# redmod-team/SympGPR

Hardware: AMD Instinct MI355X
Metric: Gram-build GB/s + Cholesky fp64 TFLOP/s at N=65536 d=2; |alpha-alpha_ref|/|alpha_ref| (higher is better)
Workload: dtype f64

## Files before the change

### include/sympgpr_probe.h

```cpp
#ifndef SYMPGPR_PROBE_H
#define SYMPGPR_PROBE_H
#include <stddef.h>
#ifdef __cplusplus
extern "C" {
#endif

int sgpr_probe_mfma_f64(int waves_per_simd, int iters, double *tflops);
int sgpr_probe_hbm_write(size_t bytes, int reps, double *gbs);
int sgpr_probe_mfma_clock(int nacc, int waves_per_simd, int iters, double *out3);
int sgpr_probe_gemm(int m, int n, int k, int lower, double *out4);
int sgpr_probe_gemm_debug(int bits);
int sgpr_probe_leaf(double *out8);
int sgpr_probe_lat(double *out8);
int sgpr_probe_xcc(int nblocks, int *host_out);
int sgpr_probe_cumask(const unsigned *mask_words, int nwords, int nblocks, int *host_out);

int sgpr_probe_generated_eval(int family, int which, int m, const double *xa, const double *ya,
                              const double *xb, const double *yb, const double *l, int nl, double *out);

int sgpr_probe_queue_plan(int n, int nworkers, int *starts_out, int max_starts, unsigned *tasks_out, int max_tasks,
                          int *counts);
int sgpr_probe_queue_plan_partial(int n, int nworkers, int nq, int *starts_out, int max_starts, unsigned *tasks_out,
                                  int max_tasks, int *counts);
int sgpr_probe_queue_trace_begin(int max_tasks);
// ... 10 lines not shown
                            double beta, double *C, size_t ldc, double alpha2, double *C2, size_t ldc2, void *stream);
int sgpr_probe_strassen2_plan(int m, int n, int k, int lower, long smin, long kslab, long smin2, long kslab2, long scratch_doubles,
                              long long *out, int max_records, int *count);
int sgpr_probe_gemm_nt4_dev(int m, int n, int k, const double *A, size_t lda, const double *B, size_t ldb, double beta, int count,
                            double *const *C, const size_t *ldc, const double *alpha, void *stream);
int sgpr_probe_strassen_rec_plan(int m, int n, int k, int lower, long scratch_doubles, long cfg_out[5], long long *out,
                                 int max_records, int *count);
int sgpr_probe_strassen_rec_scratch(int n, unsigned long long out[2]);
int sgpr_probe_gemm_strassen_rec_dev(int m, int n, int k, double alpha, const double *A, size_t lda, const double *B, size_t ldb,
                                     double beta, double *C, size_t ldc, int lower, void *stream);
int sgpr_probe_strassen_schedule(int m, int n, int k, int lower, long capacity_doubles, long long info[12], long long *out,
                                 int max_records, int *count);
int sgpr_probe_batch_layout(int path, int mode, int d, int reg, int nbatch, int n_pts, int nhyp, unsigned long long out[24]);
unsigned sgpr_probe_map_calls(void);
int sgpr_probe_map_team(int ntest, int n0);

int sgpr_probe_trsm_piece(int ticket, int cap, int strips, int out[5]);
int sgpr_probe_trsm_counts(int strips, int cap, unsigned long long out[2]);

int sgpr_probe_census(int na, int threads_a, int lds_a, int spin_a, const unsigned *mask_a, int nwords_a,
                      int nb, int threads_b, int lds_b, int spin_b, const unsigned *mask_b, int nwords_b,
                      unsigned long long *host_out);

#ifdef __cplusplus
}
#endif
#endif
```

### sympgpr_amd/_lib.py

```python
import ctypes as C
import os

import numpy as np

FAMILIES = {"A": 0, "B": 1, "C": 2, "D": 3, "USER": 4}
K_KERN, K_DXDX0, K_DYDY0, K_DXDY0 = 0, 1, 2, 3
K_DLX, K_DLY = 4, 8
K_DX, K_DY, K_DX0, K_DY0, K_DXDX0DY0, K_DYDY0DY0, K_DXDY0DY0 = 16, 17, 18, 19, 20, 21, 22
G_QQ, G_PQ, G_QP, G_PP, G_ALL, G_LOWER, G_OCML, G_DLX, G_DLY = 1, 2, 4, 8, 15, 16, 32, 64, 128
FIT_LOWER_ONLY, FIT_REG, FIT_BLOCK_QQ, FIT_BLOCK_PP = 1, 4, 8, 16
MAP_WRAP_Q, MAP_WRAP_P, MAP_EXPLICIT, MAP_LOSS_NEGP = 1, 2, 4, 8
E_ARG, E_NODEVICE, E_HIP, E_NOMEM, E_STATE = -1, -2, -3, -4, -5
LOO_LPD, LOO_PRESS = 0, 1

ABI_VERSION = 5
_dp = C.POINTER(C.c_double)
_vp = C.c_void_p


class SympGPRError(RuntimeError):
    code = None
    detail = ""


# ... 141 lines not shown
    "sgpr_probe_queue_postmortem": (C.c_int, [C.c_int]),
    "sgpr_probe_queue_force_giveup": (C.c_int, [C.c_int]),
    "sgpr_probe_tune": (C.c_int, [C.c_char_p, C.c_double]),
    "sgpr_probe_map_calls": (C.c_uint, []),
    "sgpr_probe_map_team": (C.c_int, [C.c_int, C.c_int]),
    "sgpr_probe_trsm_piece": (C.c_int, [C.c_int, C.c_int, C.c_int, C.POINTER(C.c_int)]),
    "sgpr_probe_trsm_counts": (C.c_int, [C.c_int, C.c_int, C.POINTER(C.c_ulonglong)]),
    "sgpr_probe_queue_trace_clear": (C.c_int, []),
    "sgpr_probe_strassen_plan": (C.c_int, [C.c_int, C.c_int, C.c_int, C.c_int, C.c_long, C.c_long, C.c_long,
                                           C.POINTER(C.c_longlong), C.c_int, C.POINTER(C.c_int)]),
    "sgpr_probe_gemm_strassen_dev": (C.c_int, [C.c_int, C.c_int, C.c_int, C.c_double, C.c_void_p, C.c_size_t, C.c_void_p, C.c_size_t,
                                               C.c_double, C.c_void_p, C.c_size_t, C.c_int, C.c_void_p]),
    "sgpr_probe_gemm_nt2_dev": (C.c_int, [C.c_int, C.c_int, C.c_int, C.c_double, C.c_void_p, C.c_size_t, C.c_void_p, C.c_size_t,
                                          C.c_double, C.c_void_p, C.c_size_t, C.c_double, C.c_void_p, C.c_size_t, C.c_void_p]),
    "sgpr_probe_strassen2_plan": (C.c_int, [C.c_int, C.c_int, C.c_int, C.c_int, C.c_long, C.c_long, C.c_long, C.c_long, C.c_long,
                                            C.POINTER(C.c_longlong), C.c_int, C.POINTER(C.c_int)]),
    "sgpr_probe_strassen_rec_plan": (C.c_int, [C.c_int, C.c_int, C.c_int, C.c_int, C.c_long, C.POINTER(C.c_long),
                                               C.POINTER(C.c_longlong), C.c_int, C.POINTER(C.c_int)]),
    "sgpr_probe_strassen_rec_scratch": (C.c_int, [C.c_int, C.POINTER(C.c_ulonglong)]),
    "sgpr_probe_strassen_schedule": (C.c_int, [C.c_int, C.c_int, C.c_int, C.c_int, C.c_long, C.POINTER(C.c_longlong),
                                               C.POINTER(C.c_longlong), C.c_int, C.POINTER(C.c_int)]),
    "sgpr_probe_gemm_strassen_rec_dev": (C.c_int, [C.c_int, C.c_int, C.c_int, C.c_double, C.c_void_p, C.c_size_t, C.c_void_p, C.c_size_t,
                                                   C.c_double, C.c_void_p, C.c_size_t, C.c_int, C.c_void_p]),
    "sgpr_probe_gemm_nt4_dev": (C.c_int, [C.c_int, C.c_int, C.c_int, C.c_void_p, C.c_size_t, C.c_void_p, C.c_size_t, C.c_double, C.c_int,
                                          C.POINTER(C.c_void_p), C.POINTER(C.c_size_t), C.POINTER(C.c_double), C.c_void_p]),
    "sgpr_probe_batch_layout": (C.c_int, [C.c_int, C.c_int, C.c_int, C.c_int, C.c_int, C.c_int, C.c_int,
                                          C.POINTER(C.c_ulonglong)]),
    "sgpr_probe_census": (C.c_int, [C.c_int, C.c_int, C.c_int, C.c_int, C.POINTER(C.c_uint), C.c_int,
                                    C.c_int, C.c_int, C.c_int, C.c_int, C.POINTER(C.c_uint), C.c_int,
                                    C.POINTER(C.c_ulonglong)]),
}

_LIB = None
_PROBE = None


def load_library():
    global _LIB
    if _LIB is not None:
        return _LIB
    path = lib_path()
    if os.environ.get("SYMPGPR_NO_TORCH_PRELOAD") != "1":
        try:
            import torch
        except ImportError:
            pass
# ... 78 lines not shown
```

### sympgpr_amd/csrc/chol.hip

```cpp
#include <algorithm>
#include <cstdlib>
#include <mutex>
#include <vector>

#include "cholq.h"
#include "common.h"
#include "gemm_tile.h"
#include "leaf.h"

namespace sgpr {

namespace {

using namespace leaf;


__global__ __launch_bounds__(LT) void leaf_kernel(int nb, double *A, size_t lda, double *inv,
                                                  int *dinfo, int goff, int mode,
                                                  unsigned long long *stamps)
{
    __shared__ double s[LEAF_LDS];
    if (nb == LEAF) leaf_body(s, (int)LEAF, A, lda, inv, dinfo, goff, mode, stamps);
    else            leaf_body(s, nb, A, lda, inv, dinfo, goff, mode, stamps);
}
// ... 753 lines not shown
    a.inv = q.inv + (size_t)p * q.stride_inv + (size_t)(q.k0 / (int)LEAF) * LEAF * LEAF;
    a.dinfo = q.info + p; a.goff = q.k0;
    a.flags = q.flags + (size_t)p * PFLAG_STRIDE;
    a.below_early = 1;
    (void)panel_strip(a, g, s, sh);
}

inline int split(int n)
{
    int n1 = ((n / 2 + LEAF - 1) / LEAF) * LEAF;
    if (n1 >= n) n1 -= LEAF;
    return n1;
}

struct Ctx {
    double *inv;
    int *dinfo;
    hipStream_t st;
    int la_max = 0;
    int *flags = nullptr;
    void *qws = nullptr;
    bool strassen = false;
    StrassenRec rec;
};

int potrf_lookahead(int n, double *A, size_t lda, const Ctx &c, int nb, int off0);
inline int la_block(int n) { return n <= 4096 ? 256 : (n <= 24576 ? 512 : (n <= 40960 ? 1024 : 2048)); }

int trsm_rec(int m, int n, const double *L, size_t ldl, double *B, size_t ldb, int off, const Ctx &c)
{
    if (n <= LEAF) {
        return gemm_nt(m, n, n, 1.0, B, ldb, c.inv + (size_t)(off / LEAF) * LEAF * LEAF, LEAF, 0.0,
                       B, ldb, 0, 0, c.st);
    }
    const int n1 = split(n), n2 = n - n1;
    int rc = trsm_rec(m, n1, L, ldl, B, ldb, off, c);
    if (rc) return rc;
    if (c.strassen) rc = gemm_nt_strassen_cfg(m, n2, n1, -1.0, B, ldb, L + n1, ldl, 1.0, B + (size_t)n1 * ldb, ldb, 0, strassen_rec_cfg(c.rec, n1, 0), c.st);
    else            rc = gemm_nt(m, n2, n1, -1.0, B, ldb, L + n1, ldl, 1.0, B + (size_t)n1 * ldb, ldb, 0, 0, c.st);
    if (rc) return rc;
    return trsm_rec(m, n2, L + n1 + (size_t)n1 * ldl, ldl, B + (size_t)n1 * ldb, ldb, off + n1, c);
}

int trsm_rl_rec(int m, int n, const double *L, size_t ldl, double *B, size_t ldb, int off, const Ctx &c)
{
    if (n <= LEAF)
        return gemm_nn(m, n, n, 1.0, B, ldb, c.inv + (size_t)(off / LEAF) * LEAF * LEAF, LEAF, 0.0, B, ldb, c.st);
    const int n1 = split(n), n2 = n - n1;
    int rc = trsm_rl_rec(m, n2, L + n1 + (size_t)n1 * ldl, ldl, B + (size_t)n1 * ldb, ldb, off + n1, c);
    if (rc) return rc;
    rc = gemm_nn(m, n1, n2, -1.0, B + (size_t)n1 * ldb, ldb, L + n1, ldl, 1.0, B, ldb, c.st);
    if (rc) return rc;
    return trsm_rl_rec(m, n1, L, ldl, B, ldb, off, c);
}

int potrf_rec(int n, double *A, size_t lda, int off, const Ctx &c)
{
    if (n <= LEAF) {
        hipLaunchKernelGGL(leaf_kernel, dim3(1), dim3(LT), 0, c.st, n, A, lda,
                           c.inv + (size_t)(off / LEAF) * LEAF * LEAF, c.dinfo, off, (int)LEAF_FACTOR,
                           (unsigned long long *)nullptr);
        SGPR_CHECK_LAUNCH();
        return 0;
    }
    if (n > 4 * LEAF && n <= c.la_max) return potrf_lookahead(n, A, lda, c, 0, off);
    const int n1 = split(n), n2 = n - n1;
    double *A21 = A + n1, *A22 = A + n1 + (size_t)n1 * lda;
    int rc = potrf_rec(n1, A, lda, off, c);
    if (rc) return rc;
    rc = trsm_rec(n2, n1, A, lda, A21, lda, off, c);
    if (rc) return rc;
    if (c.strassen) rc = gemm_nt_strassen_cfg(n2, n2, n1, -1.0, A21, lda, A21, lda, 1.0, A22, lda, 1, strassen_rec_cfg(c.rec, n1, 1), c.st);
    else            rc = gemm_nt(n2, n2, n1, -1.0, A21, lda, A21, lda, 1.0, A22, lda, 1, 0, c.st);
    if (rc) return rc;
    return potrf_rec(n2, A22, lda, off + n1, c);
}

int trsv_n_rec(int n, const double *L, size_t ldl, double *b, int off, const Ctx &c)
{
    if (n <= LEAF) {
        hipLaunchKernelGGL(leaf_matvec_kernel, dim3(1), dim3(MV_T), 0, c.st, n,
                           c.inv + (size_t)(off / LEAF) * LEAF * LEAF, b, 0);
        SGPR_CHECK_LAUNCH();
        return 0;
    }
    if (n <= TRSV_BLOCK) {
        hipLaunchKernelGGL(trsv_block_kernel, dim3(1), dim3(MV_T), 0, c.st, n, L, ldl,
                           c.inv + (size_t)(off / LEAF) * LEAF * LEAF, b, 0);
        SGPR_CHECK_LAUNCH();
        return 0;
    }
    const int n1 = split(n), n2 = n - n1;
    int rc = trsv_n_rec(n1, L, ldl, b, off, c);
    if (rc) return rc;
    rc = gemv_n_sub(n2, n1, L + n1, ldl, b, b + n1, c.st);
// ... 110 lines not shown
    int dev = -1;
    if (caller) {
        SGPR_HIP(hipStreamGetDevice(caller, &dev));
    } else {
        SGPR_HIP(hipGetDevice(&dev));
    }
    if (dev < 0 || dev >= 64) { set_error("potrf: device index out of range"); return SGPR_E_ARG; }
    std::lock_guard<std::mutex> lock(g_side_mu);
    if (!side[dev]) {
        int cur = -1, lo = 0, hi = 0;
        SGPR_HIP(hipGetDevice(&cur));
        if (cur != dev) SGPR_HIP(hipSetDevice(dev));
        hipError_t e = hipDeviceGetStreamPriorityRange(&lo, &hi);
        if (e == hipSuccess) e = hipStreamCreateWithPriority(&side[dev], hipStreamNonBlocking, hi);
        if (e == hipSuccess) register_exit_release();
        if (cur != dev) (void)hipSetDevice(cur);
        SGPR_HIP(e);
    }
    *out = side[dev];
    *dev_out = dev;
    return 0;
}

hipStream_t g_sum[64][2] = {};
}

int strassen_sum_streams(hipStream_t caller, int count, hipStream_t *out)
{
    int dev = -1;
    if (caller) {
        SGPR_HIP(hipStreamGetDevice(caller, &dev));
    } else {
        SGPR_HIP(hipGetDevice(&dev));
    }
    if (dev < 0 || dev >= 64 || count < 1 || count > 2) { set_error("strassen_sum_streams: bad device or count"); return SGPR_E_ARG; }
    std::lock_guard<std::mutex> lock(g_side_mu);
    for (int t = 0; t < count; ++t) {
        if (!g_sum[dev][t]) {
            int cur = -1, lo = 0, hi = 0;
            SGPR_HIP(hipGetDevice(&cur));
            if (cur != dev) SGPR_HIP(hipSetDevice(dev));
            hipError_t e = hipDeviceGetStreamPriorityRange(&lo, &hi);
            if (e == hipSuccess) e = hipStreamCreateWithPriority(&g_sum[dev][t], hipStreamNonBlocking, lo);
            if (e == hipSuccess) register_exit_release();
            if (cur != dev) (void)hipSetDevice(cur);
            SGPR_HIP(e);
        }
        out[t] = g_sum[dev][t];
    }
    return 0;
}

namespace {

struct QueueDevice {
    std::mutex mu;
    hipEvent_t done = nullptr;
    int ncu = 0;
    hipStream_t workers[4] = {}, panels[4] = {};
    bool overlap_ok[4] = {};
    bool failed = false;
};
QueueDevice g_qdev[64];

__global__ void overlap_probe_kernel(int *w, int me)
{
    __hip_atomic_store((gint *)(w + me), 1, __ATOMIC_RELAXED, __HIP_MEMORY_SCOPE_AGENT);
    const unsigned long long t0 = __builtin_amdgcn_s_memrealtime();
    int seen = 0;
    while (!(seen = __hip_atomic_load((gint *)(w + 1 - me), __ATOMIC_RELAXED, __HIP_MEMORY_SCOPE_AGENT))) {
        __builtin_amdgcn_s_sleep(32);
        if (__builtin_amdgcn_s_memrealtime() - t0 > 5000000ull) break;
// ... 122 lines not shown
    cholq::remember(ws, n, (int)(plan->tasks.size() / 2));
    cholq::remember_plan(plan);
    static const bool qdebug = tune("q_debug", 0) != 0;
    if (qdebug) {
        SGPR_HIP(hipStreamSynchronize(su));
        cholq::postmortem(false);
    }
    if (plan->nq < plan->nblk) {
        const int S = plan->starts[plan->nq];
        Ctx ct = c;
        ct.qws = nullptr;
        static const bool nosync = tune("q_nosync", 0) != 0;
        if (!nosync) SGPR_HIP(hipStreamSynchronize(su));
        return potrf_lookahead(n - S, A + S + (size_t)S * lda, lda, ct, 0, off0 + S);
    }
    return 0;
}

void release_all_streams_at_exit()
{
    int ndev = 0;
    if (hipGetDeviceCount(&ndev) != hipSuccess) { (void)hipGetLastError(); return; }
    for (int dev = 0; dev < ndev && dev < 64; ++dev) {
        hipStream_t drop[11] = {};
        int nd = 0;
        {
            std::lock_guard<std::mutex> lock(g_side_mu);
            if (g_side[dev]) { drop[nd++] = g_side[dev]; g_side[dev] = nullptr; }
            for (hipStream_t &s : g_sum[dev]) if (s) { drop[nd++] = s; s = nullptr; }
        }
        {
            QueueDevice &qd = g_qdev[dev];
            std::lock_guard<std::mutex> lock(qd.mu);
            for (int r = 0; r < 4; ++r) {
                if (qd.workers[r]) { drop[nd++] = qd.workers[r]; qd.workers[r] = nullptr; }
                if (qd.panels[r]) { drop[nd++] = qd.panels[r]; qd.panels[r] = nullptr; }
            }
            qd.failed = true;
        }
        if (!nd) continue;
        int cur = -1;
        (void)hipGetDevice(&cur);
        if (cur != dev) (void)hipSetDevice(dev);
        for (int q = 0; q < nd; ++q) (void)hipStreamDestroy(drop[q]);
        if (cur != dev && cur >= 0) (void)hipSetDevice(cur);
    }
    (void)hipGetLastError();
}

int release_streams(int dev)
{
    {
        bool any = false;
        {
            std::lock_guard<std::mutex> lock(g_side_mu);
            any = g_side[dev] != nullptr || g_sum[dev][0] != nullptr || g_sum[dev][1] != nullptr;
        }
        QueueDevice &qd = g_qdev[dev];
        std::lock_guard<std::mutex> lock(qd.mu);
        for (int r = 0; r < 4; ++r) any = any || qd.workers[r] || qd.panels[r];
        any = any || qd.done;
        if (!any) return 0;
    }
    int cur = -1;
    SGPR_HIP(hipGetDevice(&cur));
    if (cur != dev) SGPR_HIP(hipSetDevice(dev));
    hipError_t first = hipSuccess;
    auto drop = [&](hipStream_t &s) {
        if (!s) return;
        hipError_t e = hipStreamSynchronize(s);
        if (e == hipSuccess) e = hipStreamDestroy(s);
        if (e != hipSuccess && first == hipSuccess) first = e;
        s = nullptr;
    };
    {
        std::lock_guard<std::mutex> lock(g_side_mu);
        drop(g_side[dev]);
        drop(g_sum[dev][0]);
        drop(g_sum[dev][1]);
    }
    {
        QueueDevice &qd = g_qdev[dev];
        std::lock_guard<std::mutex> lock(qd.mu);
        for (int r = 0; r < 4; ++r) { drop(qd.workers[r]); drop(qd.panels[r]); }
        if (qd.done) {
            const hipError_t e = hipEventDestroy(qd.done);
            if (e != hipSuccess && first == hipSuccess) first = e;
            qd.done = nullptr;
        }
        qd.ncu = 0;
        qd.failed = false;
        for (int r = 0; r < 4; ++r) qd.overlap_ok[r] = false;
    }
    if (cur != dev) (void)hipSetDevice(cur);
    SGPR_HIP(first);
    return 0;
}

int potrf_lookahead(int n, double *A, size_t lda, const Ctx &c, int nb, int off0)
{
    if (nb == 0 && c.qws && c.flags && cholq::eligible(n) && (lda & 1) == 0 && (((uintptr_t)A & 15) == 0) && off0 % LEAF == 0) {
        const int rq = potrf_queue(n, A, lda, c, off0);
// ... 205 lines not shown
namespace {
int la_max_value()
{
    static const int v = [] { const char *e = getenv("SGPR_LA_MAX"); return (int)tune("la_max", e ? atoi(e) : 57344); }();
    return v;
}
void need_trsm(int m, int n, const StrassenRec &v, int levels, size_t &need)
{
    if (n <= LEAF || std::min(m, n) < 256) return;
    const int n1 = split(n), n2 = n - n1;
    need_trsm(m, n1, v, levels, need);
    need = std::max(need, strassen_scratch_doubles_cfg(m, n2, n1, 0, levels, strassen_rec_cfg(v, n1, 0)));
    need_trsm(m, n2, v, levels, need);
}
void need_potrf(int n, int la_max, const StrassenRec &v, int levels, size_t &need)
{
    if (n <= LEAF || (n > 4 * LEAF && n <= la_max)) return;
    const int n1 = split(n), n2 = n - n1;
    need_potrf(n1, la_max, v, levels, need);
    need_trsm(n2, n1, v, levels, need);
    need = std::max(need, strassen_scratch_doubles_cfg(n2, n2, n1, 1, levels, strassen_rec_cfg(v, n1, 1)));
    need_potrf(n2, la_max, v, levels, need);
}
}

void potrf_strassen_need(int n, size_t out[2])
{
    static const bool rec_mode = [] { const char *e = getenv("SGPR_POTRF"); return e && e[0] == 'r'; }();
    const StrassenRec v = strassen_rec_values();
    out[0] = out[1] = 0;
    need_potrf(n, rec_mode ? 0 : la_max_value(), v, 2, out[0]);
    need_potrf(n, rec_mode ? 0 : la_max_value(), v, 1, out[1]);
}

int potrf(int n, double *A, size_t lda, void *work, size_t lwork, int *dinfo, hipStream_t st)
{
    if (n < 0 || (n > 0 && lda < (size_t)n)) { set_error("potrf: bad n / lda"); return SGPR_E_ARG; }
    if (lwork < potrf_workspace(n)) { set_error("potrf: workspace too small"); return SGPR_E_ARG; }
    SGPR_HIP(hipMemsetAsync(dinfo, 0, sizeof(int), st));
    if (n == 0) return 0;
    int *flags = reinterpret_cast<int *>(static_cast<char *>(work) + inv_bytes(n));
    SGPR_HIP(hipMemsetAsync(flags, 0, flag_bytes(n), st));
    static const int mode = [] { const char *e = getenv("SGPR_POTRF"); return !e ? 0 : (e[0] == 'r' ? 1 : 2); }();
    static const int nb_env = [] { const char *e = getenv("SGPR_POTRF_NB"); return e ? atoi(e) : 0; }();
    const int la_max_env = la_max_value();
    t_last_potrf_used_queue = false;
    Ctx c{static_cast<double *>(work), dinfo, st, mode == 1 ? 0 : la_max_env, flags};
    if (cholq::ws_bytes(n) > 0) c.qws = static_cast<char *>(work) + inv_bytes(n) + flag_bytes(n) + pub_bytes(n);
    c.strassen = true;
    c.rec = strassen_rec_values();
    if (n > c.la_max && n > LEAF) {
        size_t need[2];
        potrf_strassen_need(n, need);
        strassen_reserve(need[0], need[1], st);
    }
    const bool dbg = PANEL_DBG && getenv("SGPR_PANEL_DBG") != nullptr;
    const int T = (n + LEAF - 1) / LEAF;
    if (dbg) {
        (void)hipMalloc((void **)&g_panel_dbg, sizeof(unsigned long long) * 16 * T);
        (void)hipMemset(g_panel_dbg, 0, sizeof(unsigned long long) * 16 * T);
    }
    int rc;
    if (mode == 2 || (nb_env > 0 && mode == 0 && n > 4 * LEAF && n <= c.la_max))
        rc = potrf_lookahead(n, A, lda, c, nb_env > 0 ? nb_env : 0, 0);
    else
        rc = potrf_rec(n, A, lda, 0, c);
    if (dbg) {
        (void)hipStreamSynchronize(st);
        std::vector<unsigned long long> h(16 * (size_t)T);
        (void)hipMemcpy(h.data(), g_panel_dbg, h.size() * 8, hipMemcpyDeviceToHost);
        (void)hipFree(g_panel_dbg);
        g_panel_dbg = nullptr;
        std::vector<double> d[9];
        for (int t = 1; t + 1 < T; ++t) {
            const unsigned long long *p = &h[16 * t], *q = &h[16 * (t + 1)];
            if (!p[0] || !p[5] || !q[0]) continue;
            d[0].push_back((p[1] - p[0]) * 0.01);
// ... 164 lines not shown
```

### sympgpr_amd/csrc/common.h

```cpp
#pragma once
#include <hip/hip_runtime.h>
#include <cstddef>
#include <cstdint>
#include <string>
#include <type_traits>
#include <vector>

#include "../../include/sympgpr_hip.h"

namespace sgpr {

void set_error(const std::string &msg);
double tune(const char *name, double dflt);
void tune_set(const char *name, double v);
int hip_fail(hipError_t e, const char *what, const char *file, int line);

#define SGPR_HIP(call)                                                          \
    do {                                                                        \
        hipError_t e__ = (call);                                                \
        if (e__ != hipSuccess) return ::sgpr::hip_fail(e__, #call, __FILE__, __LINE__); \
    } while (0)

#define SGPR_CHECK_LAUNCH() SGPR_HIP(hipGetLastError())

// ... 90 lines not shown
int strassen_plan(int m, int n, int k, int lower, long smin, long kslab, size_t scratch_doubles, std::vector<long long> &out);
enum { PLAN2_SUM = 4, PLAN2_PROD = 5 };
int strassen_outer_plan(int m, int n, int k, int lower, long smin, long kslab, long smin2, long kslab2, size_t scratch_doubles,
                   std::vector<long long> &out);
int gemm_nt_multi(int m, int n, int k, const double *A, size_t lda, const double *B, size_t ldb, double beta, int count,
                  double *const *C, const size_t *ldc, const double *alpha, hipStream_t st);
size_t strassen_scratch_doubles(int m, int n, int k, int lower, int levels);
struct StrassenCfg { long smin = -1, kslab = -1, smin2 = -1, kslab2 = -1, smin_under = -1; };
int gemm_nt_strassen_cfg(int m, int n, int k, double alpha, const double *A, size_t lda, const double *B, size_t ldb, double beta,
                         double *C, size_t ldc, int lower, const StrassenCfg &cfg, hipStream_t st);
size_t strassen_scratch_doubles_cfg(int m, int n, int k, int lower, int levels, const StrassenCfg &cfg);
struct StrassenRec { bool on = false; long smin_gemm = 0, smin_syrk = 0, smin2_gemm = 0, smin2_syrk = 0, kslab = 0, kslab2 = 0, kslab2_short = 0; };
StrassenRec strassen_rec_values();
StrassenCfg strassen_rec_cfg(const StrassenRec &v, int k, int lower);
int strassen_rec_plan(int m, int n, int k, int lower, long cfg_out[5], size_t scratch_doubles, std::vector<long long> &out);
int gemm_nt_strassen_rec(int m, int n, int k, double alpha, const double *A, size_t lda, const double *B, size_t ldb, double beta,
                         double *C, size_t ldc, int lower, hipStream_t st);
constexpr int SCHED_REC = 32;
int strassen_schedule(int m, int n, int k, int lower, long long cap_doubles, long long info[12], std::vector<long long> &out);
int strassen_sum_streams(hipStream_t caller, int count, hipStream_t *out);
void potrf_strassen_need(int n, size_t out[2]);
void strassen_reserve(size_t both, size_t one, hipStream_t st);
int strassen_trim();
int gemm_profile_begin();
int gemm_profile_end(double *out12);
int gemm_profile_launches(double *buf, int max_records);
void gemm_set_overlap(int on);
int gemm_nt_diag(int m, int n, int k, double alpha, const double *A, size_t lda, const double *B, size_t ldb,
                 double beta, double *C, size_t ldc, int lower, unsigned long long *stamps, int dbg, hipStream_t st);

constexpr int LEAF = 128;
constexpr int POTRF_HANDOFF_TIMEOUT = -1000001;
constexpr int SOLVE_HANDOFF_TIMEOUT = -1000002;
inline int info_status(int info)
{
    if (info >= 0) return info;
    set_error(info == POTRF_HANDOFF_TIMEOUT ? "potrf: a hand-off inside the panel kernel timed out"
              : info == SOLVE_HANDOFF_TIMEOUT ? "solve: a hand-off between the strips of a triangular solve timed out" : "potrf: internal error");
    return SGPR_E_HIP;
}
size_t potrf_workspace(int n);
int potrf(int n, double *A, size_t lda, void *work, size_t lwork, int *dinfo, hipStream_t st);
size_t potrf_batch_flag_bytes(int nbatch);
int potrf_batch_max_order();
int potrf_batch(int nbatch, int npad, double *A, size_t stride_a, size_t lda, double *inv, size_t stride_inv, int *flags,
                int *info, hipStream_t st);
// ... 122 lines not shown
```

### sympgpr_amd/csrc/gemm_f64.hip

```cpp
#include <algorithm>
#include <atomic>
#include <cstdlib>
#include <mutex>
#include <type_traits>
#include <vector>

#include "common.h"
#include "gemm_tile.h"

namespace sgpr {

namespace {

struct ProfRec { double flop; int big; int m, n, k, lower, overlap; };
struct Prof {
    std::mutex mu;
    std::atomic<bool> on{false};
    std::vector<hipEvent_t> pool;
    std::vector<ProfRec> recs;
    long dropped = 0;
};
constexpr int PROF_POOL = 8192;
Prof g_prof;
thread_local int t_overlap = 0;
// ... 915 lines not shown
size_t strassen_scratch_doubles_cfg(int m, int n, int k, int lower, int levels, const StrassenCfg &cfg)
{
    std::vector<long long> plan;
    if (!strassen_on() || m < 0 || n < 0 || k < 0 || (lower && m != n)) return 0;
    const Plan2Cfg c2 = cfg2_of(cfg, ~(size_t)0);
    if (levels >= 2 && strassen_levels() >= 2) {
        outer_plan_of(m, n, k, lower, c2, plan);
        return plan2_need(plan, c2).total();
    }
    if (strassen_plan(m, n, k, lower, c2.in.smin, c2.in.kslab, ~(size_t)0, plan)) return 0;
    return plan_need(plan);
}

void strassen_reserve(size_t both, size_t one, hipStream_t st)
{
    const int dev = device_of(st);
    if (dev < 0 || !strassen_on()) return;
    Scratch &s = g_scratch[dev];
    std::lock_guard<std::mutex> lock(s.mu);
    if (both > one && !outer_noscratch() && scratch_ensure(s, both)) return;
    if (one) (void)scratch_ensure(s, one);
}

int strassen_trim()
{
    for (Scratch &s : g_scratch) {
        std::lock_guard<std::mutex> lock(s.mu);
        if (s.p) (void)hipFree(s.p);
        if (s.ev) (void)hipEventDestroy(s.ev);
        for (hipEvent_t e : s.pool) if (e) (void)hipEventDestroy(e);
        s.pool.clear();
        s.p = nullptr; s.ev = nullptr; s.cap = 0; s.failed = 0; s.used = false; s.last = nullptr;
    }
    (void)hipGetLastError();
    return 0;
}

int gemm_nt_strassen(int m, int n, int k, double alpha, const double *A, size_t lda, const double *B, size_t ldb, double beta,
                     double *C, size_t ldc, int lower, hipStream_t st)
{
    return gemm_nt_strassen_cfg(m, n, k, alpha, A, lda, B, ldb, beta, C, ldc, lower, StrassenCfg{}, st);
}
int gemm_nt_strassen_rec(int m, int n, int k, double alpha, const double *A, size_t lda, const double *B, size_t ldb, double beta,
                         double *C, size_t ldc, int lower, hipStream_t st)
{
    return gemm_nt_strassen_cfg(m, n, k, alpha, A, lda, B, ldb, beta, C, ldc, lower, strassen_rec_cfg(strassen_rec_values(), k, lower), st);
}
int gemm_nt_strassen_cfg(int m, int n, int k, double alpha, const double *A, size_t lda, const double *B, size_t ldb, double beta,
// ... 25 lines not shown
            if (scratch_ensure(s, nd.total()))
                return enqueue(s, [&] {
                    return overlap ? run_schedule(plan, c2, nd, alpha, A, lda, B, ldb, beta, C, ldc, s, st)
                                   : run_plan2(plan, c2, nd, alpha, A, lda, B, ldb, beta, C, ldc, s.p, st);
                });
        }
    }
    rc = strassen_plan(m, n, k, lower, c2.in.smin, c2.in.kslab, ~(size_t)0, plan);
    if (rc) return rc;
    const size_t need = plan_need(plan);
    if (!need) return run_plan(plan, alpha, A, lda, B, ldb, beta, C, ldc, nullptr, nullptr, st);
    if (dev < 0) return gemm_nt(m, n, k, alpha, A, lda, B, ldb, beta, C, ldc, lower, 0, st);
    Scratch &s = g_scratch[dev];
    std::lock_guard<std::mutex> lock(s.mu);
    if (!scratch_ensure(s, need)) {
        if ((rc = strassen_plan(m, n, k, lower, c2.in.smin, c2.in.kslab, s.cap, plan))) return rc;
        if (!plan_need(plan)) return run_plan(plan, alpha, A, lda, B, ldb, beta, C, ldc, nullptr, nullptr, st);
    }
    const Need2 nd = plan2_need(plan, c2);
    if (overlap) return enqueue(s, [&] { return run_schedule(plan, c2, nd, alpha, A, lda, B, ldb, beta, C, ldc, s, st); });
    return enqueue(s, [&] { return run_plan(plan, alpha, A, lda, B, ldb, beta, C, ldc, s.p, s.p + nd.v[0], st); });
}

}
```

### sympgpr_amd/csrc/probe.hip

```cpp
#include <algorithm>
#include <cstdlib>
#include <vector>

#include "cholq.h"
#include "common.h"
#include "../../include/sympgpr_probe.h"
#include "generated/pair_generated.h"
#include "nd_eval.h"

namespace sgpr {
namespace {
typedef double double4_t __attribute__((ext_vector_type(4)));
typedef double double2_t __attribute__((ext_vector_type(2)));

template <int NACC>
__global__ __launch_bounds__(256) void mfma_clock_kernel(int iters, double *out, unsigned long long *stamps)
{
    double4_t acc[NACC];
    const double a = 1.0 + threadIdx.x * 1e-9, b = 1.0 - threadIdx.x * 1e-9;
#pragma unroll
    for (int i = 0; i < NACC; ++i) acc[i] = double4_t{0.0, 0.0, 0.0, 0.0};
    const unsigned long long t0 = __builtin_amdgcn_s_memtime(), r0 = __builtin_amdgcn_s_memrealtime();
    for (int it = 0; it < iters; ++it) {
#pragma unroll
// ... 529 lines not shown
    return 0;
}
extern "C" int sgpr_probe_strassen_schedule(int m, int n, int k, int lower, long capacity_doubles, long long info[12], long long *out,
                                            int max_records, int *count)
{
    if (!count) { set_error("probe_strassen_schedule: bad arguments"); return SGPR_E_ARG; }
    std::vector<long long> sched;
    const int rc = strassen_schedule(m, n, k, lower, (long long)capacity_doubles, info, sched);
    if (rc) return rc;
    *count = (int)(sched.size() / SCHED_REC);
    for (size_t i = 0; out && i < sched.size() && (int)(i / SCHED_REC) < max_records; ++i) out[i] = sched[i];
    return 0;
}
extern "C" int sgpr_probe_gemm_strassen_rec_dev(int m, int n, int k, double alpha, const double *A, size_t lda, const double *B, size_t ldb,
                                                double beta, double *C, size_t ldc, int lower, void *stream)
{
    return gemm_nt_strassen_rec(m, n, k, alpha, A, lda, B, ldb, beta, C, ldc, lower, static_cast<hipStream_t>(stream));
}
extern "C" int sgpr_probe_gemm_nt4_dev(int m, int n, int k, const double *A, size_t lda, const double *B, size_t ldb, double beta,
                                       int count, double *const *C, const size_t *ldc, const double *alpha, void *stream)
{
    return gemm_nt_multi(m, n, k, A, lda, B, ldb, beta, count, C, ldc, alpha, static_cast<hipStream_t>(stream));
}
extern "C" int sgpr_probe_batch_layout(int path, int mode, int d, int reg, int nbatch, int n_pts, int nhyp, unsigned long long out[24])
{
    const long n = d ? 2L * d * n_pts : reg ? (long)n_pts : 2L * n_pts;
    if (path < 0 || path > 1 || mode < 0 || mode > 3 || (path && mode == 3) || d < 0 || d > 3 || (d && (reg || mode > 1)) || nbatch < 1 ||
        n_pts < 1 || nhyp < 1 || (path ? n <= 256 || n > 2048 : n > 256) || !out) {
        set_error("probe_batch_layout: bad arguments");
        return SGPR_E_ARG;
    }
    const BatchLayout l = batch_layout(path, mode, d, reg, nbatch, n_pts, nhyp);
    const size_t v[24] = {(size_t)l.chunk, l.nacc, l.o_x, l.o_y, l.o_z, l.o_kc, l.o_no, l.in_bytes, l.o_al, l.o_nll, l.o_info, l.out_bytes,
                          l.o_A, l.o_inv, l.o_fl, l.o_fl2, l.o_r, l.o_pub, l.o_st, l.o_part, l.scr_bytes,
                          sizeof(KConst), sizeof(nd::NdConst), l.flag_bytes};
    for (int i = 0; i < 24; ++i) out[i] = v[i];
    return 0;
}
extern "C" unsigned sgpr_probe_map_calls(void) { return applymap_last_calls(); }
extern "C" int sgpr_probe_map_team(int ntest, int n0) { return applymap_team(ntest, n0); }
extern "C" int sgpr_probe_trsm_piece(int ticket, int cap, int strips, int out[5]) { if (ticket < 0 || cap < 1 || strips < 0 || !out) return SGPR_E_ARG; trsm_piece_of(ticket, cap, strips, out); return 0; }
extern "C" int sgpr_probe_trsm_counts(int strips, int cap, unsigned long long out[2])
{
    if (strips < 0 || cap < 1 || !out) return SGPR_E_ARG;
    size_t c[2];
    trsm_piece_counts(strips, cap, c);
// ... 51 lines not shown
```

Before: 82.32.

## Add a third Strassen level at the top of recursive Cholesky updates

Adds an extra Strassen recursion level on top of the existing two-level recursive Strassen GEMM used in the recursive potrf/trsm trailing updates. Large operands are split into halves with k-slabs, and the seven products go into a scratch buffer that is then accumulated into C. Operand sums run on a low-priority side stream with double-buffered scratch, so they can overlap the products. The aim is to cut fp64 multiply count at N=65536, at the cost of extra memory traffic for sums and accumulation, more scratch memory, and some loss of numerical accuracy.

```diff
diff --git a/include/sympgpr_probe.h b/include/sympgpr_probe.h
--- a/include/sympgpr_probe.h
+++ b/include/sympgpr_probe.h
@@ -56,6 +56,12 @@
                       int nb, int threads_b, int lds_b, int spin_b, const unsigned *mask_b, int nwords_b,
                       unsigned long long *host_out);
 
+int sgpr_probe_strassen_top_plan(int m, int n, int k, int lower, long scratch_doubles, long long *out, int max_records, int *count);
+int sgpr_probe_strassen_cfg_plan(int m, int n, int k, int lower, const long cfg[5], long long *out, int max_records, int *count);
+int sgpr_probe_strassen_top_scratch(int n, unsigned long long out[2]);
+int sgpr_probe_gemm_strassen_top_dev(int m, int n, int k, double alpha, const double *A, size_t lda, const double *B, size_t ldb,
+                                     double beta, double *C, size_t ldc, int lower, void *stream);
+
 #ifdef __cplusplus
 }
 #endif
diff --git a/sympgpr_amd/_lib.py b/sympgpr_amd/_lib.py
--- a/sympgpr_amd/_lib.py
+++ b/sympgpr_amd/_lib.py
@@ -187,6 +187,13 @@
                                                C.POINTER(C.c_longlong), C.c_int, C.POINTER(C.c_int)]),
     "sgpr_probe_gemm_strassen_rec_dev": (C.c_int, [C.c_int, C.c_int, C.c_int, C.c_double, C.c_void_p, C.c_size_t, C.c_void_p, C.c_size_t,
                                                    C.c_double, C.c_void_p, C.c_size_t, C.c_int, C.c_void_p]),
+    "sgpr_probe_strassen_top_plan": (C.c_int, [C.c_int, C.c_int, C.c_int, C.c_int, C.c_long, C.POINTER(C.c_longlong), C.c_int,
+                                               C.POINTER(C.c_int)]),
+    "sgpr_probe_strassen_cfg_plan": (C.c_int, [C.c_int, C.c_int, C.c_int, C.c_int, C.POINTER(C.c_long), C.POINTER(C.c_longlong), C.c_int,
+                                               C.POINTER(C.c_int)]),
+    "sgpr_probe_strassen_top_scratch": (C.c_int, [C.c_int, C.POINTER(C.c_ulonglong)]),
+    "sgpr_probe_gemm_strassen_top_dev": (C.c_int, [C.c_int, C.c_int, C.c_int, C.c_double, C.c_void_p, C.c_size_t, C.c_void_p, C.c_size_t,
+                                                   C.c_double, C.c_void_p, C.c_size_t, C.c_int, C.c_void_p]),
     "sgpr_probe_gemm_nt4_dev": (C.c_int, [C.c_int, C.c_int, C.c_int, C.c_void_p, C.c_size_t, C.c_void_p, C.c_size_t, C.c_double, C.c_int,
                                           C.POINTER(C.c_void_p), C.POINTER(C.c_size_t), C.POINTER(C.c_double), C.c_void_p]),
     "sgpr_probe_batch_layout": (C.c_int, [C.c_int, C.c_int, C.c_int, C.c_int, C.c_int, C.c_int, C.c_int,
diff --git a/sympgpr_amd/csrc/chol.hip b/sympgpr_amd/csrc/chol.hip
--- a/sympgpr_amd/csrc/chol.hip
+++ b/sympgpr_amd/csrc/chol.hip
@@ -799,6 +799,7 @@
     void *qws = nullptr;
     bool strassen = false;
     StrassenRec rec;
+    StrassenTop top;
 };
 
 int potrf_lookahead(int n, double *A, size_t lda, const Ctx &c, int nb, int off0);
@@ -813,7 +814,7 @@
     const int n1 = split(n), n2 = n - n1;
     int rc = trsm_rec(m, n1, L, ldl, B, ldb, off, c);
     if (rc) return rc;
-    if (c.strassen) rc = gemm_nt_strassen_cfg(m, n2, n1, -1.0, B, ldb, L + n1, ldl, 1.0, B + (size_t)n1 * ldb, ldb, 0, strassen_rec_cfg(c.rec, n1, 0), c.st);
+    if (c.strassen) rc = strassen_top_gemm(m, n2, n1, -1.0, B, ldb, L + n1, ldl, 1.0, B + (size_t)n1 * ldb, ldb, 0, &c.rec, &c.top, c.st);
     else            rc = gemm_nt(m, n2, n1, -1.0, B, ldb, L + n1, ldl, 1.0, B + (size_t)n1 * ldb, ldb, 0, 0, c.st);
     if (rc) return rc;
     return trsm_rec(m, n2, L + n1 + (size_t)n1 * ldl, ldl, B + (size_t)n1 * ldb, ldb, off + n1, c);
@@ -847,7 +848,7 @@
     if (rc) return rc;
     rc = trsm_rec(n2, n1, A, lda, A21, lda, off, c);
     if (rc) return rc;
-    if (c.strassen) rc = gemm_nt_strassen_cfg(n2, n2, n1, -1.0, A21, lda, A21, lda, 1.0, A22, lda, 1, strassen_rec_cfg(c.rec, n1, 1), c.st);
+    if (c.strassen) rc = strassen_top_gemm(n2, n2, n1, -1.0, A21, lda, A21, lda, 1.0, A22, lda, 1, &c.rec, &c.top, c.st);
     else            rc = gemm_nt(n2, n2, n1, -1.0, A21, lda, A21, lda, 1.0, A22, lda, 1, 0, c.st);
     if (rc) return rc;
     return potrf_rec(n2, A22, lda, off + n1, c);
@@ -1004,7 +1005,7 @@
     return 0;
 }
 
-hipStream_t g_sum[64][2] = {};
+hipStream_t g_sum[64][3] = {};
 }
 
 int strassen_sum_streams(hipStream_t caller, int count, hipStream_t *out)
@@ -1030,6 +1031,30 @@
         }
         out[t] = g_sum[dev][t];
     }
+    return 0;
+}
+
+int strassen_top_stream(hipStream_t caller, hipStream_t *out)
+{
+    int dev = -1;
+    if (caller) {
+        SGPR_HIP(hipStreamGetDevice(caller, &dev));
+    } else {
+        SGPR_HIP(hipGetDevice(&dev));
+    }
+    if (dev < 0 || dev >= 64 || !out) { set_error("strassen_top_stream: bad device"); return SGPR_E_ARG; }
+    std::lock_guard<std::mutex> lock(g_side_mu);
+    if (!g_sum[dev][2]) {
+        int cur = -1, lo = 0, hi = 0;
+        SGPR_HIP(hipGetDevice(&cur));
+        if (cur != dev) SGPR_HIP(hipSetDevice(dev));
+        hipError_t e = hipDeviceGetStreamPriorityRange(&lo, &hi);
+        if (e == hipSuccess) e = hipStreamCreateWithPriority(&g_sum[dev][2], hipStreamNonBlocking, lo);
+        if (e == hipSuccess) register_exit_release();
+        if (cur != dev) (void)hipSetDevice(cur);
+        SGPR_HIP(e);
+    }
+    *out = g_sum[dev][2];
     return 0;
 }
 
@@ -1198,7 +1223,7 @@
     int ndev = 0;
     if (hipGetDeviceCount(&ndev) != hipSuccess) { (void)hipGetLastError(); return; }
     for (int dev = 0; dev < ndev && dev < 64; ++dev) {
-        hipStream_t drop[11] = {};
+        hipStream_t drop[12] = {};
         int nd = 0;
         {
             std::lock_guard<std::mutex> lock(g_side_mu);
@@ -1230,7 +1255,7 @@
         bool any = false;
         {
             std::lock_guard<std::mutex> lock(g_side_mu);
-            any = g_side[dev] != nullptr || g_sum[dev][0] != nullptr || g_sum[dev][1] != nullptr;
+            any = g_side[dev] != nullptr || g_sum[dev][0] != nullptr || g_sum[dev][1] != nullptr || g_sum[dev][2] != nullptr;
         }
         QueueDevice &qd = g_qdev[dev];
         std::lock_guard<std::mutex> lock(qd.mu);
@@ -1254,6 +1279,7 @@
         drop(g_side[dev]);
         drop(g_sum[dev][0]);
         drop(g_sum[dev][1]);
+        drop(g_sum[dev][2]);
     }
     {
         QueueDevice &qd = g_qdev[dev];
@@ -1505,6 +1531,33 @@
     need = std::max(need, strassen_scratch_doubles_cfg(n2, n2, n1, 1, levels, strassen_rec_cfg(v, n1, 1)));
     need_potrf(n2, la_max, v, levels, need);
 }
+void need3_trsm(int m, int n, const StrassenRec &v, const StrassenTop &t, size_t &need)
+{
+    if (n <= LEAF || std::min(m, n) / 2 < t.smin3) return;
+    const int n1 = split(n), n2 = n - n1;
+    need3_trsm(m, n1, v, t, need);
+    need = std::max(need, strassen_top_scratch_doubles(m, n2, n1, 0, v, t));
+    need3_trsm(m, n2, v, t, need);
+}
+void need3_potrf(int n, int la_max, const StrassenRec &v, const StrassenTop &t, size_t &need)
+{
+    if (n <= LEAF || (n > 4 * LEAF && n <= la_max)) return;
+    const int n1 = split(n), n2 = n - n1;
+    need3_potrf(n1, la_max, v, t, need);
+    need3_trsm(n2, n1, v, t, need);
+    need = std::max(need, strassen_top_scratch_doubles(n2, n2, n1, 1, v, t));
+    need3_potrf(n2, la_max, v, t, need);
+}
+}
+
+size_t potrf_strassen_top_need(int n)
+{
+    static const bool rec_mode = [] { const char *e = getenv("SGPR_POTRF"); return e && e[0] == 'r'; }();
+    const StrassenRec v = strassen_rec_values();
+    const StrassenTop t = strassen_top_values();
+    size_t need = 0;
+    if (v.on && t.smin3 > 0) need3_potrf(n, rec_mode ? 0 : la_max_value(), v, t, need);
+    return need;
 }
 
 void potrf_strassen_need(int n, size_t out[2])
@@ -1532,10 +1585,12 @@
     if (cholq::ws_bytes(n) > 0) c.qws = static_cast<char *>(work) + inv_bytes(n) + flag_bytes(n) + pub_bytes(n);
     c.strassen = true;
     c.rec = strassen_rec_values();
+    c.top = strassen_top_values();
     if (n > c.la_max && n > LEAF) {
         size_t need[2];
         potrf_strassen_need(n, need);
         strassen_reserve(need[0], need[1], st);
+        strassen_top_reserve(potrf_strassen_top_need(n), st);
     }
     const bool dbg = PANEL_DBG && getenv("SGPR_PANEL_DBG") != nullptr;
     const int T = (n + LEAF - 1) / LEAF;
diff --git a/sympgpr_amd/csrc/common.h b/sympgpr_amd/csrc/common.h
--- a/sympgpr_amd/csrc/common.h
+++ b/sympgpr_amd/csrc/common.h
@@ -136,6 +136,18 @@
 void potrf_strassen_need(int n, size_t out[2]);
 void strassen_reserve(size_t both, size_t one, hipStream_t st);
 int strassen_trim();
+enum { PLAN3_SUM = 6, PLAN3_ZERO = 7, PLAN3_PROD = 8, PLAN3_ACC = 9, PLAN3_PASS = 10 };
+struct StrassenTop { long smin3 = 0, kslab3 = 0, kslab3_short = 0; };
+StrassenTop strassen_top_values();
+int strassen_top_plan(int m, int n, int k, int lower, const StrassenRec *v, const StrassenTop *t, size_t scratch_doubles,
+                      std::vector<long long> &out);
+int strassen_cfg_plan(int m, int n, int k, int lower, const long cfg[5], std::vector<long long> &out);
+size_t strassen_top_scratch_doubles(int m, int n, int k, int lower, const StrassenRec &v, const StrassenTop &t);
+int strassen_top_gemm(int m, int n, int k, double alpha, const double *A, size_t lda, const double *B, size_t ldb, double beta,
+                      double *C, size_t ldc, int lower, const StrassenRec *v, const StrassenTop *t, hipStream_t st);
+size_t potrf_strassen_top_need(int n);
+void strassen_top_reserve(size_t need, hipStream_t st);
+int strassen_top_stream(hipStream_t caller, hipStream_t *out);
 int gemm_profile_begin();
 int gemm_profile_end(double *out12);
 int gemm_profile_launches(double *buf, int max_records);
diff --git a/sympgpr_amd/csrc/gemm_f64.hip b/sympgpr_amd/csrc/gemm_f64.hip
--- a/sympgpr_amd/csrc/gemm_f64.hip
+++ b/sympgpr_amd/csrc/gemm_f64.hip
@@ -961,8 +961,11 @@
     if (one) (void)scratch_ensure(s, one);
 }
 
+namespace { void top_trim(); }
+
 int strassen_trim()
 {
+    top_trim();
     for (Scratch &s : g_scratch) {
         std::lock_guard<std::mutex> lock(s.mu);
         if (s.p) (void)hipFree(s.p);
@@ -1034,4 +1037,320 @@
     return enqueue(s, [&] { return run_plan(plan, alpha, A, lda, B, ldb, beta, C, ldc, s.p, s.p + nd.v[0], st); });
 }
 
-}
+namespace {
+constexpr long REC_SMIN3 = 16384, REC_KSLAB3 = 65536, REC_KSLAB3_SHORT = 32768;
+
+__global__ __launch_bounds__(256) void block_acc_kernel(int rows, int cols, const double *T, double *C1, double a1, double *C2, double a2,
+                                                        size_t ldc)
+{
+    const int nrc = (rows + 511) / 512, ncg = (cols + 3) / 4;
+    const long pieces = (long)nrc * ncg;
+    for (long p = blockIdx.x; p < pieces; p += gridDim.x) {
+        const int cg = (int)(p / nrc), rc = (int)(p - (long)cg * nrc);
+        const int r = rc * 512 + 2 * (int)threadIdx.x;
+        if (r >= rows) continue;
+        double2_t t[4], c1[4], c2[4];
+#pragma unroll
+        for (int u = 0; u < 4; ++u) {
+            const int c = min(cg * 4 + u, cols - 1);
+            t[u] = *reinterpret_cast<const double2_t *>(T + (size_t)r + (size_t)c * (size_t)rows);
+            c1[u] = *reinterpret_cast<const double2_t *>(C1 + (size_t)r + (size_t)c * ldc);
+            if (C2) c2[u] = *reinterpret_cast<const double2_t *>(C2 + (size_t)r + (size_t)c * ldc);
+        }
+#pragma unroll
+        for (int u = 0; u < 4; ++u) {
+            const int c = cg * 4 + u;
+            if (c >= cols) continue;
+            *reinterpret_cast<double2_t *>(C1 + (size_t)r + (size_t)c * ldc) = c1[u] + a1 * t[u];
+            if (C2) *reinterpret_cast<double2_t *>(C2 + (size_t)r + (size_t)c * ldc) = c2[u] + a2 * t[u];
+        }
+    }
+}
+int block_acc(int rows, int cols, const double *T, double *C1, double a1, double *C2, double a2, size_t ldc, hipStream_t st, long wgs)
+{
+    const long pieces = (long)((rows + 511) / 512) * ((cols + 3) / 4);
+    hipLaunchKernelGGL(block_acc_kernel, dim3((unsigned)std::min(pieces, wgs)), dim3(256), 0, st, rows, cols, T, C1, a1, C2, a2, ldc);
+    SGPR_CHECK_LAUNCH();
+    return 0;
+}
+
+long top_slab(long k, const StrassenTop &t)
+{
+    const long s = (t.kslab3 > 0 && k >= t.kslab3) ? t.kslab3 : t.kslab3_short;
+    return (s >= 128 && s % 128 == 0 && k >= s) ? s : 0;
+}
+bool top_qualifies(long m, long n, long k, const StrassenRec &v, const StrassenTop &t, size_t scratch)
+{
+    if (!v.on || t.smin3 <= 0 || m <= 0 || n <= 0 || m % 2048 != 0 || n % 1024 != 0) return false;
+    if (m / 2 < t.smin3 || n / 2 < t.smin3) return false;
+    const long slab = top_slab(k, t);
+    return slab && (size_t)(m / 2) * (size_t)(n / 2) + (size_t)(m / 2 + n / 2) * (size_t)(slab / 2) <= scratch;
+}
+void put_cfg(std::vector<long long> &out, int at, const StrassenCfg &c)
+{
+    long long *r = &out[out.size() - STRASSEN_REC + at];
+    r[0] = c.smin; r[1] = c.kslab; r[2] = c.smin2; r[3] = c.kslab2; r[4] = c.smin_under;
+}
+void top_pass(int lower, long ar, long ac, long br, long bc, long m, long n, long k, long cr, long cc, int kind, const StrassenRec &v,
+              std::vector<long long> &out)
+{
+    put(out, {PLAN3_PASS, lower, ar, ac, br, bc, m, n, k, cr, cc});
+    put_cfg(out, 11, strassen_rec_cfg(v, (int)k, kind));
+}
+void top_gemm(long m, long n, long k, long ar, long br, long cr, long cc, int kind, const StrassenRec &v, const StrassenTop &t,
+              size_t scratch, std::vector<long long> &out)
+{
+    if (!top_qualifies(m, n, k, v, t, scratch)) { top_pass(0, ar, 0, br, 0, m, n, k, cr, cc, kind, v, out); return; }
+    const long slab = top_slab(k, t), m2 = m / 2, n2 = n / 2, k2 = slab / 2;
+    std::vector<long long> seven_recs;
+    long k0 = 0;
+    for (; k0 + slab <= k; k0 += slab) {
+        seven_recs.clear();
+        seven(PLAN3_SUM, PLAN3_PROD, m2, n2, k2, k0, ar, br, cr, cc, seven_recs);
+        for (size_t i = 0; i + STRASSEN_REC <= seven_recs.size(); i += STRASSEN_REC) {
+            const long long *r = &seven_recs[i];
+            if (r[0] == PLAN3_SUM) { out.insert(out.end(), r, r + STRASSEN_REC); continue; }
+            put(out, {PLAN3_ZERO, m2, n2});
+            put(out, {PLAN3_PROD, r[1], r[2], r[3], r[4], r[5], r[6], r[7], r[8], r[9]});
+            put_cfg(out, 10, strassen_rec_cfg(v, (int)k2, kind));
+            put(out, {PLAN3_ACC, m2, n2, r[10], r[11], r[12], r[13], r[14], r[15]});
+        }
+    }
+    if (k0 < k) top_pass(0, ar, k0, br, k0, m, n, k - k0, cr, cc, kind, v, out);
+}
+void top_syrk(long n, long k, const StrassenRec &v, const StrassenTop &t, size_t scratch, std::vector<long long> &out)
+{
+    const long h = n / 2;
+    if (n % 2 != 0 || !top_qualifies(h, h, k, v, t, scratch)) { top_pass(1, 0, 0, 0, 0, n, n, k, 0, 0, 1, v, out); return; }
+    top_pass(1, 0, 0, 0, 0, h, h, k, 0, 0, 1, v, out);
+    top_gemm(h, h, k, h, 0, h, 0, 1, v, t, scratch, out);
+    top_pass(1, h, 0, h, 0, h, h, k, h, h, 1, v, out);
+}
+struct Need3 { size_t v[3] = {0, 0, 0}; size_t total() const { return v[0] + v[1] + v[2]; } };
+Need3 top_need(const std::vector<long long> &plan)
+{
+    Need3 nd;
+    for (size_t i = 0; i + STRASSEN_REC <= plan.size(); i += STRASSEN_REC) {
+        const long long *r = &plan[i];
+        if (r[0] == PLAN3_ZERO) nd.v[0] = std::max(nd.v[0], (size_t)r[1] * (size_t)r[2]);
+        else if (r[0] == PLAN3_SUM) nd.v[1 + r[1]] = std::max(nd.v[1 + r[1]], (size_t)r[2] * (size_t)r[3]);
+    }
+    return nd;
+}
+
+struct TopScratch {
+    std::mutex mu;
+    double *p = nullptr;
+    size_t cap = 0, failed = 0;
+    hipEvent_t ev = nullptr;
+    hipStream_t last = nullptr;
+    bool used = false;
+    std::vector<hipEvent_t> pool;
+};
+TopScratch g_top[64];
+
+int top_buffers_wanted() { return (tune("rec_strassen3_overlap", 1) != 0 && tune("rec_strassen3_buffers", 2) >= 2) ? 2 : 1; }
+bool top_ensure(TopScratch &s, size_t need, int sets)
+{
+    if (tune("rec_strassen3_noscratch", 0) != 0) return false;
+    if (s.cap >= need) return true;
+    if (s.failed && need >= s.failed) return false;
+    if (s.p) { (void)hipFree(s.p); s.p = nullptr; s.cap = 0; s.used = false; }
+    for (int b = sets; b >= 1; --b) {
+        const size_t want = need * (size_t)b;
+        if (s.failed && want >= s.failed) continue;
+        if (hipMalloc((void **)&s.p, want * sizeof(double)) == hipSuccess) { s.cap = want; return true; }
+        (void)hipGetLastError();
+        s.p = nullptr;
+        s.failed = want;
+    }
+    return false;
+}
+void top_trim()
+{
+    for (TopScratch &s : g_top) {
+        std::lock_guard<std::mutex> lock(s.mu);
+        if (s.p) (void)hipFree(s.p);
+        if (s.ev) (void)hipEventDestroy(s.ev);
+        for (hipEvent_t e : s.pool) if (e) (void)hipEventDestroy(e);
+        s.pool.clear();
+        s.p = nullptr; s.ev = nullptr; s.cap = 0; s.failed = 0; s.used = false; s.last = nullptr;
+    }
+    (void)hipGetLastError();
+}
+
+int run_top(const std::vector<long long> &plan, const Need3 &nd, double alpha, const double *A, size_t lda, const double *B, size_t ldb,
+            double *C, size_t ldc, TopScratch &s, hipStream_t st)
+{
+    const size_t need = nd.total();
+    const bool overlap = tune("rec_strassen3_overlap", 1) != 0;
+    const int nbuf = (top_buffers_wanted() >= 2 && s.cap >= 2 * need) ? 2 : 1;
+    const long wgs = overlap ? std::min(65535L, std::max(1L, (long)tune("gemm_strassen_sum_wgs", (double)SUM_WGS_SIDE))) : SUM_WGS;
+    hipStream_t sd = st;
+    int rc = 0;
+    if (overlap && (rc = strassen_top_stream(st, &sd))) return rc;
+    auto at = [&](int region, int b) { return s.p + (size_t)b * need + (region == 0 ? 0 : (region == 1 ? nd.v[0] : nd.v[0] + nd.v[1])); };
+    auto event = [&](size_t i) {
+        if (s.pool.size() <= i) s.pool.resize(i + 1, nullptr);
+        if (!s.pool[i]) SGPR_HIP(hipEventCreateWithFlags(&s.pool[i], hipEventDisableTiming));
+        return 0;
+    };
+    auto join = [&]() {
+        if (!overlap) return 0;
+        SGPR_HIP(hipEventRecord(s.pool[1], sd));
+        SGPR_HIP(hipStreamWaitEvent(st, s.pool[1], 0));
+        return 0;
+    };
+    struct Join {
+        bool on; hipStream_t sd, st; hipEvent_t ev;
+        ~Join()
+        {
+            if (on && (hipEventRecord(ev, sd) != hipSuccess || hipStreamWaitEvent(st, ev, 0) != hipSuccess)) {
+                (void)hipGetLastError();
+                (void)hipStreamSynchronize(sd);
+            }
+        }
+    };
+    if ((rc = event(0)) || (rc = event(1))) return rc;
+    if (overlap) {
+        SGPR_HIP(hipEventRecord(s.pool[0], st));
+        SGPR_HIP(hipStreamWaitEvent(sd, s.pool[0], 0));
+    }
+    Join at_exit{overlap, sd, st, s.pool[1]};
+    struct Pend { const long long *r; int b; size_t p; };
+    std::vector<Pend> pending;
+    size_t p = 0;
+    auto flush = [&]() {
+        for (const Pend &q : pending) {
+            const long long *r = q.r;
+            if (overlap) SGPR_HIP(hipStreamWaitEvent(sd, s.pool[3 + 2 * q.p], 0));
+            const int e = block_acc((int)r[1], (int)r[2], at(0, q.b), C + r[3] + (size_t)r[4] * ldc, alpha * (double)r[5],
+                                    r[8] ? C + r[6] + (size_t)r[7] * ldc : nullptr, alpha * (double)r[8], ldc, sd, wgs);
+            if (e) return e;
+        }
+        pending.clear();
+        return 0;
+    };
+    for (size_t i = 0; i + STRASSEN_REC <= plan.size(); i += STRASSEN_REC) {
+        const long long *r = &plan[i];
+        const int b = (int)(p % (size_t)nbuf);
+        if (r[0] == PLAN3_SUM) {
+            if (nbuf == 1 && (rc = flush())) return rc;
+            const double *P = r[1] ? B : A;
+            const size_t ld = r[1] ? ldb : lda;
+            rc = block_sum((int)r[2], (int)r[3], P + r[4] + (size_t)r[5] * ld, ld, P + r[6] + (size_t)r[7] * ld, ld, (double)r[8],
+                           at(1 + (int)r[1], b), sd, wgs);
+        } else if (r[0] == PLAN3_ZERO) {
+            if (nbuf == 1 && (rc = flush())) return rc;
+            SGPR_HIP(hipMemsetAsync(at(0, b), 0, (size_t)r[1] * (size_t)r[2] * sizeof(double), sd));
+        } else if (r[0] == PLAN3_PROD) {
+            const int m = (int)r[7], n = (int)r[8], k = (int)r[9];
+            if (overlap) {
+                if ((rc = event(2 + 2 * p)) || (rc = event(3 + 2 * p))) return rc;
+                SGPR_HIP(hipEventRecord(s.pool[2 + 2 * p], sd));
+                SGPR_HIP(hipStreamWaitEvent(st, s.pool[2 + 2 * p], 0));
+            }
+            const double *X = r[1] ? at(1, b) : A + r[2] + (size_t)r[3] * lda;
+            const double *Y = r[4] ? at(2, b) : B + r[5] + (size_t)r[6] * ldb;
+            StrassenCfg cfg;
+            cfg.smin = (long)r[10]; cfg.kslab = (long)r[11]; cfg.smin2 = (long)r[12]; cfg.kslab2 = (long)r[13]; cfg.smin_under = (long)r[14];
+            rc = gemm_nt_strassen_cfg(m, n, k, 1.0, X, r[1] ? (size_t)m : lda, Y, r[4] ? (size_t)n : ldb, 1.0, at(0, b), (size_t)m, 0, cfg, st);
+            if (rc) return rc;
+            if (overlap) SGPR_HIP(hipEventRecord(s.pool[3 + 2 * p], st));
+            rc = flush();
+        } else if (r[0] == PLAN3_ACC) {
+            pending.push_back(Pend{r, b, p});
+            ++p;
+        } else if (r[0] == PLAN3_PASS) {
+            if ((rc = flush()) || (rc = join())) return rc;
+            StrassenCfg cfg;
+            cfg.smin = (long)r[11]; cfg.kslab = (long)r[12]; cfg.smin2 = (long)r[13]; cfg.kslab2 = (long)r[14]; cfg.smin_under = (long)r[15];
+            rc = gemm_nt_strassen_cfg((int)r[6], (int)r[7], (int)r[8], alpha, A + r[2] + (size_t)r[3] * lda, lda, B + r[4] + (size_t)r[5] * ldb, ldb,
+                                      1.0, C + r[9] + (size_t)r[10] * ldc, ldc, (int)r[1], cfg, st);
+        } else {
+            set_error("run_top: unknown record");
+            rc = SGPR_E_ARG;
+        }
+        if (rc) return rc;
+    }
+    return flush();
+}
+}
+
+StrassenTop strassen_top_values()
+{
+    StrassenTop t;
+    t.smin3 = std::max(0L, (long)tune("rec_strassen3_min", (double)REC_SMIN3));
+    t.kslab3 = std::max(0L, (long)tune("rec_strassen3_kslab", (double)REC_KSLAB3));
+    t.kslab3_short = std::max(0L, (long)tune("rec_strassen3_kslab_short", (double)REC_KSLAB3_SHORT));
+    return t;
+}
+
+int strassen_top_plan(int m, int n, int k, int lower, const StrassenRec *vp, const StrassenTop *tp, size_t scratch_doubles,
+                      std::vector<long long> &out)
+{
+    const StrassenRec v = vp ? *vp : strassen_rec_values();
+    const StrassenTop t = tp ? *tp : strassen_top_values();
+    if (m < 0 || n < 0 || k < 0 || (lower && m != n)) { set_error("strassen_top_plan: bad extents"); return SGPR_E_ARG; }
+    out.clear();
+    if (lower) top_syrk(n, k, v, t, scratch_doubles, out);
+    else       top_gemm(m, n, k, 0, 0, 0, 0, 0, v, t, scratch_doubles, out);
+    return 0;
+}
+int strassen_cfg_plan(int m, int n, int k, int lower, const long cfg[5], std::vector<long long> &out)
+{
+    if (m < 0 || n < 0 || k < 0 || (lower && m != n) || !cfg) { set_error("strassen_cfg_plan: bad arguments"); return SGPR_E_ARG; }
+    StrassenCfg c;
+    c.smin = cfg[0]; c.kslab = cfg[1]; c.smin2 = cfg[2]; c.kslab2 = cfg[3]; c.smin_under = cfg[4];
+    outer_plan_of(m, n, k, lower, cfg2_of(c, ~(size_t)0), out);
+    return 0;
+}
+size_t strassen_top_scratch_doubles(int m, int n, int k, int lower, const StrassenRec &v, const StrassenTop &t)
+{
+    std::vector<long long> plan;
+    if (strassen_levels() < 2 || strassen_top_plan(m, n, k, lower, &v, &t, ~(size_t)0, plan)) return 0;
+    return top_need(plan).total();
+}
+void strassen_top_reserve(size_t need, hipStream_t st)
+{
+    const int dev = device_of(st);
+    if (dev < 0 || !need) return;
+    TopScratch &s = g_top[dev];
+    std::lock_guard<std::mutex> lock(s.mu);
+    if (s.cap >= need * (size_t)top_buffers_wanted()) return;
+    if (s.cap >= need && s.failed && need * 2 >= s.failed) return;
+    if (s.p) { (void)hipFree(s.p); s.p = nullptr; s.cap = 0; s.used = false; }
+    (void)top_ensure(s, need, top_buffers_wanted());
+}
+
+int strassen_top_gemm(int m, int n, int k, double alpha, const double *A, size_t lda, const double *B, size_t ldb, double beta,
+                      double *C, size_t ldc, int lower, const StrassenRec *vp, const StrassenTop *tp, hipStream_t st)
+{
+    const StrassenRec v = vp ? *vp : strassen_rec_values();
+    const StrassenTop t = tp ? *tp : strassen_top_values();
+    const StrassenCfg cfg = strassen_rec_cfg(v, k, lower);
+    const bool aligned = ((((uintptr_t)A | (uintptr_t)B | (uintptr_t)C) & 15) == 0) && (((lda | ldb | ldc) & 1) == 0);
+    const int dev = (!v.on || t.smin3 <= 0 || std::min(lower ? m / 2 : m, lower ? n / 2 : n) / 2 < t.smin3) ? -1 : device_of(st);
+    if (dev < 0 || strassen_levels() < 2 || !aligned || beta != 1.0 || (lower && m != n))
+        return gemm_nt_strassen_cfg(m, n, k, alpha, A, lda, B, ldb, beta, C, ldc, lower, cfg, st);
+    std::vector<long long> plan;
+    int rc = strassen_top_plan(m, n, k, lower, &v, &t, ~(size_t)0, plan);
+    if (rc) return rc;
+    const Need3 nd = top_need(plan);
+    if (nd.total()) {
+        TopScratch &s = g_top[dev];
+        std::lock_guard<std::mutex> lock(s.mu);
+        if (top_ensure(s, nd.total(), top_buffers_wanted())) {
+            if (!s.ev) SGPR_HIP(hipEventCreateWithFlags(&s.ev, hipEventDisableTiming));
+            if (s.used && s.last != st) SGPR_HIP(hipStreamWaitEvent(st, s.ev, 0));
+            rc = run_top(plan, nd, alpha, A, lda, B, ldb, C, ldc, s, st);
+            SGPR_HIP(hipEventRecord(s.ev, st));
+            s.last = st;
+            s.used = true;
+            return rc;
+        }
+    }
+    return gemm_nt_strassen_cfg(m, n, k, alpha, A, lda, B, ldb, beta, C, ldc, lower, cfg, st);
+}
+
+}
diff --git a/sympgpr_amd/csrc/probe.hip b/sympgpr_amd/csrc/probe.hip
--- a/sympgpr_amd/csrc/probe.hip
+++ b/sympgpr_amd/csrc/probe.hip
@@ -575,6 +575,38 @@
 {
     return gemm_nt_multi(m, n, k, A, lda, B, ldb, beta, count, C, ldc, alpha, static_cast<hipStream_t>(stream));
 }
+extern "C" int sgpr_probe_strassen_top_plan(int m, int n, int k, int lower, long scratch_doubles, long long *out, int max_records, int *count)
+{
+    if (!count || scratch_doubles < 0) { set_error("probe_strassen_top_plan: bad arguments"); return SGPR_E_ARG; }
+    std::vector<long long> plan;
+    const int rc = strassen_top_plan(m, n, k, lower, nullptr, nullptr, (size_t)scratch_doubles, plan);
+    if (rc) return rc;
+    *count = (int)(plan.size() / STRASSEN_REC);
+    for (size_t i = 0; out && i < plan.size() && (int)(i / STRASSEN_REC) < max_records; ++i) out[i] = plan[i];
+    return 0;
+}
+extern "C" int sgpr_probe_strassen_cfg_plan(int m, int n, int k, int lower, const long cfg[5], long long *out, int max_records, int *count)
+{
+    if (!count) { set_error("probe_strassen_cfg_plan: bad arguments"); return SGPR_E_ARG; }
+    std::vector<long long> plan;
+    const int rc = strassen_cfg_plan(m, n, k, lower, cfg, plan);
+    if (rc) return rc;
+    *count = (int)(plan.size() / STRASSEN_REC);
+    for (size_t i = 0; out && i < plan.size() && (int)(i / STRASSEN_REC) < max_records; ++i) out[i] = plan[i];
+    return 0;
+}
+extern "C" int sgpr_probe_strassen_top_scratch(int n, unsigned long long out[2])
+{
+    if (n < 0 || !out) { set_error("probe_strassen_top_scratch: bad arguments"); return SGPR_E_ARG; }
+    out[0] = potrf_strassen_top_need(n);
+    out[1] = 2 * out[0];
+    return 0;
+}
+extern "C" int sgpr_probe_gemm_strassen_top_dev(int m, int n, int k, double alpha, const double *A, size_t lda, const double *B, size_t ldb,
+                                                double beta, double *C, size_t ldc, int lower, void *stream)
+{
+    return strassen_top_gemm(m, n, k, alpha, A, lda, B, ldb, beta, C, ldc, lower, nullptr, nullptr, static_cast<hipStream_t>(stream));
+}
 extern "C" int sgpr_probe_batch_layout(int path, int mode, int d, int reg, int nbatch, int n_pts, int nhyp, unsigned long long out[24])
 {
     const long n = d ? 2L * d * n_pts : reg ? (long)n_pts : 2L * n_pts;
```

Result: faster. 84.62, median of 6 (+2.8%).
